# Intel-HLS/GenomicsDB

Hardware: AMD Instinct MI355X
Metric: combined-gVCF positions/sec (higher is better)
Workload: dtype u8/int32

## Files before the change

### __graft_entry__.py

```python
import os
import sys

ROOT = os.path.dirname(os.path.abspath(__file__))
sys.path.insert(0, ROOT)
sys.path.insert(0, os.path.join(ROOT, "tests"))


def build():
    from genomicsdb_amd import build as b
    lib = b.build_native(verbose=True)
    b.build_oracle()
    b.build_hostsim()
    b.build_hostsim_variants()
    b.build_hostsim_import()
    b.build_hostsim_inflate()
    b.build_hostsim_import_bcf()
    b.build_hostsim_import_csv()
    b.build_hostsim_dispatch()
    b.build_hostsim_merge()
    b.build_hostsim_merge_files()
    b.build_hostsim_split()
    b.build_hostsim_histogram()
    b.build_hostsim_index()
    b.build_hostsim_vcfdiff()
    b.build_hostsim_import_stream()
    b.build_hostsim_columns()
    b.build_jni_importer_harness()
    from genomicsdb_amd import synth
    synth.lib()
    import genomicsdb_amd
    from genomicsdb_amd import _lib
    L = _lib.lib()
    for s in _lib.SYMBOLS:
        getattr(L, s)
    print("built", lib)


def smoke():
    import helpers
    from golden_cases import CASES
    import genomicsdb_amd
    case = [c for c in CASES if c[0] == "t6_7_8_vcf_at_0"][0]
    name, callsets, vid, ov, golden, mode = case
    cells = helpers.cells_for(callsets, vid)
    q, pb = helpers.query_json(callsets, vid, ov, mode)
    want, _, _ = helpers.oracle_run(q, cells)
    s = genomicsdb_amd.GenomicsDBQueryStream(query_json=q, cells=cells, buffer_capacity=4096)
    got = s.read()
    s.close()
    assert got == want, "device output differs from the oracle"
    assert got == helpers.golden_text(golden)
    print("smoke ok: %d bytes, bit-exact vs oracle and reference golden" % len(got))


if __name__ == "__main__":
    build()
    if len(sys.argv) > 1 and sys.argv[1] == "smoke":
        smoke()
```

### genomicsdb_amd/build.py

```python
import os
import subprocess
import sys

PKG = os.path.dirname(os.path.abspath(__file__))
ROOT = os.path.dirname(PKG)
CSRC = os.path.join(PKG, "csrc")
OBJ = os.path.join(ROOT, "build", "obj")
LIB = os.path.join(PKG, "libgenomicsdb_amd.so")
TOOL = os.path.join(PKG, "gt_mpi_gather")
TOOLS = {"gt_mpi_gather": TOOL, "vcf2tiledb": os.path.join(PKG, "vcf2tiledb"), "test_genomicsdb_importer": os.path.join(PKG, "test_genomicsdb_importer"),
         "vcf_histogram": os.path.join(PKG, "vcf_histogram"), "vcfdiff": os.path.join(PKG, "vcfdiff")}

SOURCES = [
    "kernels/gdb_pipeline.hip",
    "kernels/gdb_bgzf.hip",
    "kernels/gdb_import.hip",
    "kernels/gdb_import_stream.hip",
    "kernels/gdb_inflate.hip",
    "kernels/gdb_merge.hip",
    "kernels/gdb_split.hip",
    "kernels/gdb_histogram.hip",
    "kernels/gdb_index.hip",
    "kernels/gdb_vcfdiff.hip",
    "kernels/gdb_columns.hip",
# ... 149 lines not shown
    d = os.path.join(ROOT, "tests", "hostsim_index")
    subprocess.check_call(["make", "-s", "-C", d])
    return os.path.join(d, "libhostsim_index.so"), os.path.join(d, "hostsim_index")


def build_hostsim_vcfdiff():
    d = os.path.join(ROOT, "tests", "hostsim_vcfdiff")
    subprocess.check_call(["make", "-s", "-C", d])
    return os.path.join(d, "hostsim_vcfdiff")


def build_hostsim_columns():
    d = os.path.join(ROOT, "tests", "hostsim_columns")
    subprocess.check_call(["make", "-s", "-C", d])
    return os.path.join(d, "libhostsim_columns.so"), os.path.join(d, "hostsim_columns_main")


def build_hostsim_inflate():
    subprocess.check_call(["make", "-s", "-C", os.path.join(ROOT, "tests", "hostsim_inflate")])
    return os.path.join(ROOT, "tests", "hostsim_inflate", "libhostsim_inflate.so")


def build_hostsim_tile_inflate():
    d = os.path.join(ROOT, "tests", "hostsim_tile_inflate")
    subprocess.check_call(["make", "-s", "-C", d])
    return os.path.join(d, "libhostsim_tile_inflate.so"), os.path.join(d, "tile_inflate_fuzz")


def build_hostsim_dispatch():
    subprocess.check_call(["make", "-s", "-C", os.path.join(ROOT, "tests", "hostsim_dispatch")])
    return os.path.join(ROOT, "tests", "hostsim_dispatch", "libhostsim_dispatch.so")


if __name__ == "__main__":
    print(build_native(verbose=True))
    print(build_oracle())
```

### genomicsdb_amd/csrc/core/gdb_stages.hpp

```cpp
#pragma once
#include "gdb_core.hpp"

#if defined(__HIP_DEVICE_COMPILE__)
#define GDB_ATOMIC_ADD_I32(p, v) atomicAdd((int*)(p), (int)(v))
#define GDB_ATOMIC_OR_U32(p, v) atomicOr((unsigned*)(p), (unsigned)(v))
#define GDB_ATOMIC_ADD_U64(p, v) atomicAdd((unsigned long long*)(p), (unsigned long long)(v))
#else
#define GDB_ATOMIC_ADD_I32(p, v) (*(p) += (v))
#define GDB_ATOMIC_OR_U32(p, v) (*(p) |= (v))
#define GDB_ATOMIC_ADD_U64(p, v) (*(p) += (uint64_t)(v))
#endif

#define GDB_EVENT_SENTINEL 0xFFFFFFFFFFFFFFFFull

GDB_HD void stage_eff_end(const FragmentView& fr, const CellMeta& cm, const int64_t* perm, int64_t j, int64_t* rm_begin, int64_t* span, uint32_t* err) {
  const int64_t C = fr.ncells;
  const int64_t c = perm[j];
  int64_t eff = fr.end[c];
  if (j + 1 < C) {
    const int64_t nx = perm[j + 1];
    if (fr.row[nx] == fr.row[c] && fr.begin[nx] <= eff) {
      eff = fr.begin[nx] - 1;
      if (!(cm.cflags[c] & (GDB_CF_DELETION | GDB_CF_REFBLOCK))) *err |= GDB_ERR_OVERLAP_NOT_REFBLOCK_OR_DELETION;
    }
// ... 128 lines not shown
    keys[base + (k - klo)] = (uint64_t)k * (uint64_t)nrows + (uint64_t)fr.row[c];
    vals[base + (k - klo)] = c;
  }
  (void)lut_len;
}
GDB_HD int64_t stage_heavy_base(const uint64_t* sorted_keys, int64_t T, int64_t nrows, int64_t k) {
  const uint64_t want = (uint64_t)k * (uint64_t)nrows;
  int64_t lo = 0, hi = T;
  while (lo < hi) { int64_t mid = (lo + hi) >> 1; if (sorted_keys[mid] < want) lo = mid + 1; else hi = mid; }
  return lo;
}

struct RowIndex {
  const int64_t* row_ptr;
  const int64_t* rm_cell;
  const int64_t* rm_begin;
};
struct RowWalker {
  int64_t j, j_begin, j_end;
  GDB_HD void init(const RowIndex& ri, int32_t row, int64_t s0) {
    j_begin = ri.row_ptr[row]; j_end = ri.row_ptr[row + 1];
    int64_t lo = j_begin, hi = j_end;
    while (lo < hi) { int64_t mid = (lo + hi) >> 1; if (ri.rm_begin[mid] <= s0) lo = mid + 1; else hi = mid; }
    j = lo - 1;
  }
  GDB_HD int64_t live(const RowIndex& ri, const CellMeta& cm, int64_t s) {
    while (j + 1 < j_end && ri.rm_begin[j + 1] <= s) ++j;
    if (j < j_begin) return -1;
    const int64_t c = ri.rm_cell[j];
    return (s <= cm.eff_end[c]) ? c : -1;
  }
};

GDB_HD RecordInfo load_record_info(const SiteOut& so, const HeavyLists& hl, int64_t k) {
  RecordInfo ri;
  ri.num_merged = so.num_alleles[k];
  ri.rflags = so.rflags[k];
  ri.fmt_mask = so.fmt_mask[k];
  ri.hbase = hl.base[k];
  ri.hend = hl.base[k + 1];
  return ri;
}
```

### genomicsdb_amd/csrc/kernels/gdb_assembly_choice.hpp

```cpp
#pragma once
#include <algorithm>
#include <cstdint>
#include <cstdlib>

namespace genomicsdb_amd {

constexpr int kAsmRows = 64;
constexpr int kWaveLds = 8 * 1024;
constexpr int kCooperativeEntry = 512;

enum { kSizeKernelPlain = 0, kSizeKernel3x8 = 1, kSizeKernel3x16 = 2, kSizeKernelPieces = 3, kSizeKernelEvents = 4 };
enum { kPageKernelWrite = 1, kPageKernelWrite2 = 2, kPageKernelWrite3 = 3, kPageKernelEvents = 4, kPageKernelBcf = 5 };
constexpr int page_kernel_code(int size_kernel, int page_kernel, int waves, int coop_u, int lds_bytes) {
  return size_kernel * 100000 + page_kernel * 10000 + waves * 1000 + coop_u * 100 + lds_bytes / 1024;
}

struct AssemblyKnobs {
  int run, run_w, run_w2, run_f;
  uint64_t resolved_budget_bytes;
  bool events; int ev_run;
  int asm_path;
  int size3_rounds;
  bool size3_check;
  bool res_compact;
  bool res_chunk_major;
  int write_waves;
  bool write_image_set; int write_image_kb;
  int order_block_log2;
  bool coop_unroll, xcd_aware;
  int page_priority;

  int image_kb(uint64_t avg_chunk_bytes) const { return write_image_set ? write_image_kb : avg_chunk_bytes && avg_chunk_bytes <= 3400 ? 4 : 8; }
  bool page_priority_on(bool engine_asks) const { return page_priority >= 0 ? page_priority == 1 : engine_asks; }
};

typedef const char* (*KnobLookup)(const char* name);

inline bool res_layout_chunk_major(KnobLookup get) { const char* e = get("GDBAMD_RES_LAYOUT"); return e && *e == '1'; }

inline AssemblyKnobs read_assembly_knobs(KnobLookup get) {
  const auto num = [get](const char* name, int unset, int lo, int hi) { const char* e = get(name); return e && *e ? std::max(lo, std::min(hi, atoi(e))) : unset; };
  const auto on = [get](const char* name) { const char* e = get(name); return e && *e && *e != '0'; };
  const auto not_off = [get](const char* name) { const char* e = get(name); return !(e && *e == '0'); };
  const int any = 0x7fffffff;
  AssemblyKnobs k{};
  const int size3 = num("GDBAMD_SIZE3", 8, -any, any);
  k.size3_rounds = size3 == 0 ? 0 : size3 >= 16 ? 16 : 8;
  k.run = num("GDBAMD_RUN", k.size3_rounds ? 128 : 64, 1, any);
  k.run_w = num("GDBAMD_RUN_W", 32, 1, any);
  k.run_w2 = num("GDBAMD_RUN_W2", 64, 1, any);
  k.run_f = num("GDBAMD_RUN_F", 128, 1, any);
  const char* mb = get("GDBAMD_RESOLVED_MB");
  k.resolved_budget_bytes = mb && *mb ? (uint64_t)atoll(mb) << 20 : (uint64_t)32 << 30;
  k.events = on("GDBAMD_EVENTS");
  k.ev_run = num("GDBAMD_EV_RUN", 32, 1, 64);
  k.asm_path = num("GDBAMD_ASM_PATH", 0, 0, 3);
  k.size3_check = on("GDBAMD_SIZE3_CHECK");
  k.res_compact = !k.size3_check && not_off("GDBAMD_RES_COMPACT");
  k.res_chunk_major = res_layout_chunk_major(get);
  k.write_waves = num("GDBAMD_WRITE_WAVES", 1, -any, any);
  const char* image = get("GDBAMD_WRITE_IMAGE_KB");
  k.write_image_set = image && *image;
  k.write_image_kb = k.write_image_set ? atoi(image) : 0;
  k.order_block_log2 = num("GDBAMD_ORDER_BLOCK_LOG2", 12, 0, 30);
  k.coop_unroll = not_off("GDBAMD_COOP_UNROLL");
  k.xcd_aware = not_off("GDBAMD_XCD_AWARE");
  const char* prio = get("GDBAMD_PAGE_PRIORITY");
  k.page_priority = prio && (*prio == '0' || *prio == '1') ? *prio - '0' : -1;
  return k;
}

inline int size_kernel_for(const AssemblyKnobs& k, int run) {
  return k.size3_rounds == 0 || run > 64 * 1024 ? kSizeKernelPlain : k.size3_rounds >= 16 ? kSizeKernel3x16 : kSizeKernel3x8;
}

struct IntervalFacts { bool bcf_mode; int64_t P; int32_t N; bool untabled_records, any_over255; };

struct AssemblySizing {
  bool bcf_mode;
  int asm_path;
  bool piece_path;
  int size_kernel;
  int run, frun, evrun;
  bool use_events;
  bool resolved_whole;
  bool res_compact;
  bool chunk_major;
  int resolved_entry_bytes;
  int64_t res_rows(int64_t rows) const { return chunk_major ? rows : 0; }
};

inline AssemblySizing choose_sizing(const AssemblyKnobs& k, const IntervalFacts& f) {
  AssemblySizing s{};
  s.bcf_mode = f.bcf_mode;
  const uint64_t nchunks = (uint64_t)((f.N + kAsmRows - 1) / kAsmRows), entry = 8;
  s.asm_path = k.events ? 0 : (f.bcf_mode && (k.asm_path & 1)) ? 2 : k.asm_path;
  if (s.asm_path == 3 && f.untabled_records) s.asm_path = 0;
  s.piece_path = s.asm_path == 1 || s.asm_path == 3;
  s.run = k.run; s.frun = k.run_f; s.evrun = k.ev_run;
  const bool events_fit_blocks = k.events && ((1 << k.order_block_log2) % k.ev_run) == 0;
  s.resolved_whole = !s.piece_path && (f.bcf_mode || ((uint64_t)f.P * nchunks * kAsmRows * entry <= k.resolved_budget_bytes && !events_fit_blocks));
// ... 55 lines not shown
```

### genomicsdb_amd/csrc/kernels/gdb_pipeline.hip

```cpp
#include <hip/hip_runtime.h>

#include <fcntl.h>
#include <sys/stat.h>
#include <unistd.h>
#include <zlib.h>

#include <algorithm>
#include <cstdio>
#include <cstdlib>
#include <chrono>
#include <cstring>
#include <memory>
#include <mutex>
#include <thread>
#include <vector>

#include <rocprim/device/device_radix_sort.hpp>
#include <rocprim/device/device_reduce.hpp>
#include <rocprim/device/device_scan.hpp>
#include <rocprim/iterator/reverse_iterator.hpp>

#include "../core/gdb_stages.hpp"
#include "../core/gdb_bcf.hpp"
#include "../core/gdb_calls.hpp"
// ... 1132 lines not shown
  const bool is_long = l > inline_max;
  if (desc) desc[s] = is_long ? make_uint2(kOverflowBit | ovf16[s], l) : make_uint2((uint32_t)s * (kSlotStride / 16), l);
  if (tag_pool && (is_long || l == 0u)) *reinterpret_cast<uint2*>(tag_pool + (size_t)s * kSlotStride + kSlotTagAt) = make_uint2(is_long ? (kOverflowBit | ovf16[s]) : 0u, l);
}

struct __attribute__((aligned(16))) WalkCell {
  int64_t eff_end;
  uint64_t aux;
  int32_t k_lo, k_hi;
  uint32_t base;
  uint32_t flags;
};
constexpr uint32_t kWalkHeavy = 1u;
constexpr int kWalkChunksShift = 1;
constexpr uint32_t kWalkChunksMask = 7u;
__device__ __forceinline__ uint32_t inline_chunks(uint32_t len) { return len <= (uint32_t)kInlineText ? min((len + 15u) >> 4, kWalkChunksMask) : 0u; }
__global__ void k_walk_static(const int64_t* perm, const int32_t* row, const int64_t* row_ptr, int32_t N, const int64_t* eff_end, const uint32_t* cflags, int64_t C, WalkCell* walk, int64_t* inv) {
  const int64_t j = (int64_t)blockIdx.x * blockDim.x + threadIdx.x;
  WalkCell w;
  w.aux = 0; w.k_lo = -1; w.k_hi = -1; w.base = 0;
  if (j < C) {
    const int64_t c = perm[j];
    const int64_t at = j + row[c];
    w.eff_end = eff_end[c]; w.flags = (cflags[c] & GDB_CF_HEAVY) ? kWalkHeavy : 0u;
    walk[at] = w;
    inv[c] = at;
  } else if (j < C + N) {
    const int64_t r = j - C;
    w.eff_end = INT64_MIN; w.flags = 0;
    walk[row_ptr[r + 1] + r] = w;
  }
}
__global__ void k_walk_window(const int64_t* inv, const uint32_t* cflags, const int64_t* hoff, const int32_t* k_lo, const int32_t* k_hi, const uint32_t* tbase, const uint64_t* tmask,
                              const uint32_t* slot_len, uint32_t light_base, uint32_t heavy_base, int64_t c_base, int64_t n, uint32_t epoch, WalkCell* walk) {
  const int64_t i = (int64_t)blockIdx.x * blockDim.x + threadIdx.x;
  if (i >= n) return;
  const int64_t c = c_base + i;
  WalkCell* w = walk + inv[c];
  const bool heavy = (cflags[c] & GDB_CF_HEAVY) != 0;
  uint32_t chunks = 0;
  if (k_lo[c] >= 0) {
    const uint32_t first = heavy ? heavy_base + (uint32_t)hoff[i] : light_base + tbase[i];
    const uint32_t cnt = heavy ? (uint32_t)(k_hi[c] - k_lo[c] + 1) : (uint32_t)__popcll(tmask[i]);
    for (uint32_t q = 0; q < cnt; ++q) chunks = max(chunks, inline_chunks(slot_len[first + q]));
  }
  const uint4 tail = make_uint4((uint32_t)k_lo[c], (uint32_t)k_hi[c], heavy ? (uint32_t)hoff[i] : tbase[i], (epoch << 8) | (chunks << kWalkChunksShift) | (heavy ? kWalkHeavy : 0u));
  w->aux = heavy ? 0ull : tmask[i];
  *reinterpret_cast<uint4*>(&w->k_lo) = tail;
}

struct AsmCtx {
  const int64_t* row_ptr;
  const int64_t* rm_begin;
  const WalkCell* walk;
  const int64_t* rec_start;
  const uint8_t* rtype;
  const uint32_t* prefix_len;
  const uint2* desc;
  const char* pool;
  const uint32_t* ubase;
  uint32_t light_base, heavy_base, row_base;
  int32_t nrows;
};

struct SlotWalker {
  int64_t j, j_end, next_begin, cur_end;
  uint64_t aux;
  uint32_t base;
  int32_t k_lo, row_;
  bool heavy;
  __device__ __forceinline__ void load(const AsmCtx& a) {
    const WalkCell w = a.walk[j + row_];
    next_begin = (j + 1 < j_end) ? a.rm_begin[j + 1] : INT64_MAX;
    cur_end = w.eff_end; aux = w.aux; base = w.base; k_lo = w.k_lo; heavy = (w.flags & kWalkHeavy) != 0;
  }
  __device__ __forceinline__ void init(const AsmCtx& a, int32_t row, int64_t s0) {
    row_ = row;
    const int64_t j_begin = a.row_ptr[row];
    j_end = a.row_ptr[row + 1];
    int64_t lo = j_begin, hi = j_end;
    while (lo < hi) { const int64_t mid = (lo + hi) >> 1; if (a.rm_begin[mid] <= s0) lo = mid + 1; else hi = mid; }
    j = lo - 1;
    if (j >= j_begin) load(a);
    else { cur_end = INT64_MIN; heavy = false; aux = 0; base = 0; k_lo = 0; next_begin = (j + 1 < j_end) ? a.rm_begin[j + 1] : INT64_MAX; }
  }
  __device__ __forceinline__ void advance(const AsmCtx& a, int64_t s) { while (next_begin <= s) { ++j; load(a); } }
  __device__ __forceinline__ uint32_t slot(const AsmCtx& a, int64_t k, int64_t s, uint32_t t, int32_t row) const {
    const bool dead = s > cur_end;
    if (!dead && heavy) return a.heavy_base + base + (uint32_t)(k - (int64_t)k_lo);
    if (t == kUntabledType) return a.row_base + a.ubase[k] * (uint32_t)a.nrows + (uint32_t)row;
    if (dead) return t;
    return a.light_base + base + (uint32_t)__popcll(aux & ((1ull << t) - 1ull));
  }
};

__device__ __forceinline__ void settle_loads() { __builtin_amdgcn_s_waitcnt(0x0F70); }
struct SlotCopy {
  gdb_lds_char* dst;
  __attribute__((address_space(3))) uint32_t* dw;
  __attribute__((address_space(3))) uint32_t* scrap;
  uint32_t n, h, nw, carry, head_word;
  __device__ __forceinline__ void begin(gdb_lds_char* d, uint32_t len, gdb_lds_char* scrap_word) {
    dst = d; n = len;
    h = (4u - ((uint32_t)(uintptr_t)d & 3u)) & 3u;
    if (h > n) h = n;
    nw = (n - h + 3u) >> 2;
    dw = (__attribute__((address_space(3))) uint32_t*)(d + h);
    scrap = (__attribute__((address_space(3))) uint32_t*)scrap_word;
    carry = 0; head_word = 0;
  }
  __device__ __forceinline__ void put(uint32_t m, uint32_t v) const { *((m < nw) ? dw + m : scrap) = v; }
  __device__ __forceinline__ void chunk(uint32_t q, const uint4& x) {
    if (q == 0) head_word = x.x;
    const uint32_t m1 = q << 2;
    put(m1 - 1u, __builtin_amdgcn_alignbyte(x.x, carry, h));
// ... 37 lines not shown
  __device__ __forceinline__ uint2 load(int64_t at) const {
    if (off) return make_uint2(off[at], (uint32_t)len8[at]);
    return wide[at];
  }
};
__global__ void __launch_bounds__(kAsmRows)
k_assemble_size(AsmCtx a, const int32_t* __restrict__ order, int64_t n, int32_t N, int nchunks, int run, uint64_t* __restrict__ chunk_size,
                ResMatrix resolved, int64_t resolved_base, int64_t res_rows) {
  const int64_t ib = (int64_t)(blockIdx.x / (unsigned)nchunks) * run;
  const int64_t ie = min(n, ib + (int64_t)run);
  const int ch = (int)(blockIdx.x % (unsigned)nchunks);
  const int lane = threadIdx.x;
  const int32_t r = ch * kAsmRows + lane;
  SlotWalker w;
  int64_t prev_k = INT64_MAX;
  uint32_t cur_slot = kNoSlot;
  uint2 cur = make_uint2(0, 0);
  for (int64_t i0 = ib; i0 < ie; i0 += 64) {
    const int cnt = (int)min((int64_t)64, ie - i0);
    int32_t my_k = 0; int64_t my_s = 0; uint32_t my_t = 0; uint64_t my_total = 0;
    if (lane < cnt) {
      my_k = order[i0 + lane];
      my_s = a.rec_start[my_k];
      my_t = a.rtype[my_k];
      if (ch == 0) my_total = a.prefix_len[my_k];
      if (ch == nchunks - 1) my_total += 1;
    }
    for (int jj = 0; jj < cnt; ++jj) {
      const int64_t k = __builtin_amdgcn_readlane(my_k, jj);
      const int64_t s = readlane64(my_s, jj);
      const uint32_t t = (uint32_t)__builtin_amdgcn_readlane((int)my_t, jj);
      uint2 d = make_uint2(0, 0);
      if (r < N) {
        if (k < prev_k) w.init(a, r, s); else w.advance(a, s);
        const uint32_t sl = w.slot(a, k, s, t, r);
        if (sl != cur_slot) { cur_slot = sl; cur = a.desc[sl]; }
        d = cur;
      }
      prev_k = k;
      if (resolved.any()) resolved.store(res_row(k - resolved_base, ch, nchunks, res_rows) * kAsmRows + lane, d);
      const uint32_t total = wave_total(wave_inclusive_scan_dpp(d.y));
      if (lane == jj) my_total += total;
    }
    if (chunk_size && lane < cnt) chunk_size[(int64_t)my_k * nchunks + ch] = my_total;
  }
}

#ifdef GDBAMD_SIZE3_WAVES
#define GDBAMD_SIZE3_ATTR __attribute__((amdgpu_waves_per_eu(GDBAMD_SIZE3_WAVES)))
#else
#define GDBAMD_SIZE3_ATTR
#endif
template <int R> __global__ void __launch_bounds__(kAsmRows) GDBAMD_SIZE3_ATTR
k_assemble_size3(AsmCtx a, const int32_t* __restrict__ order, int64_t n, int32_t N, int nchunks, int run, uint64_t* __restrict__ chunk_size,
                 ResMatrix resolved, int64_t resolved_base, int64_t res_rows) {
  __shared__ int64_t ss[kAsmRows];
  __shared__ int32_t ks[kAsmRows];
  __shared__ uint32_t diff[kAsmRows + 1];
  __shared__ uint2 pl_d[R * kAsmRows];
  __shared__ uint8_t pl_at[R * kAsmRows];
  const int64_t ib = (int64_t)(blockIdx.x / (unsigned)nchunks) * run;
  const int64_t ie = min(n, ib + (int64_t)run);
  const int ch = (int)(blockIdx.x % (unsigned)nchunks);
  const int lane = threadIdx.x;
  const int32_t r = ch * kAsmRows + lane;
  const bool has_row = r < N;
  SlotWalker w;
  int64_t prev_k = INT64_MAX;
  uint32_t cur_slot = kNoSlot;
  uint2 cur = make_uint2(0, 0);
  for (int64_t i0 = ib; i0 < ie; i0 += 64) {
    const int cnt = (int)min((int64_t)64, ie - i0);
    int32_t my_k = 0; int64_t my_s = INT64_MAX; uint32_t my_t = 0; uint64_t my_total = 0;
    if (lane < cnt) {
      my_k = order[i0 + lane];
      my_s = a.rec_start[my_k];
      my_t = a.rtype[my_k];
      if (ch == 0) my_total = a.prefix_len[my_k];
      if (ch == nchunks - 1) my_total += 1;
    }
    ss[lane] = my_s; ks[lane] = my_k; diff[lane] = 0u;
    if (lane == 0) diff[kAsmRows] = 0u;
    const int32_t left_k = __shfl_up(my_k, 1, 64);
    const uint32_t left_t = (uint32_t)__shfl_up((int)my_t, 1, 64);
    const uint64_t heads = __ballot(lane < cnt && (lane == 0 || my_k < left_k || my_t != left_t));
    __builtin_amdgcn_fence(__ATOMIC_SEQ_CST, "wavefront");
    for (int seg_a = 0; seg_a < cnt;) {
      const uint64_t behind = seg_a + 1 < 64 ? heads >> (seg_a + 1) : 0ull;
      const int seg_b = behind ? seg_a + 1 + (int)__builtin_ctzll(behind) : cnt;
      const int64_t k_a = __builtin_amdgcn_readlane(my_k, seg_a);
      const uint32_t t = (uint32_t)__builtin_amdgcn_readlane((int)my_t, seg_a);
      if (k_a < prev_k && has_row) w.init(a, r, readlane64(my_s, seg_a));
      for (int ra = seg_a; ra < seg_b; ra += R) {
        const int rb = min(seg_b, ra + R);
        int pos = ra, np = 0;
        while (__any((int)(pos < rb))) {
          if (pos < rb) {
            uint2 d = make_uint2(0, 0);
            int e = rb;
            if (has_row) {
              const int64_t s = ss[pos];
              const int64_t k = ks[pos];
              w.advance(a, s);
              const uint32_t sl = w.slot(a, k, s, t, r);
              if (sl != cur_slot) { cur_slot = sl; cur = a.desc[sl]; }
              d = cur;
              const bool dead = s > w.cur_end;
              if (t == kUntabledType || (!dead && w.heavy)) e = pos + 1;
              else {
                const int64_t x = dead ? w.next_begin - 1 : min(w.cur_end, w.next_begin - 1);
                int lo = pos + 1, hi = rb;
                while (lo < hi) { const int mid = (lo + hi) >> 1; if (ss[mid] > x) hi = mid; else lo = mid + 1; }
                e = lo;
              }
            }
            pl_d[np * kAsmRows + lane] = d;
            pl_at[np * kAsmRows + lane] = (uint8_t)pos;
            ++np;
            if (chunk_size && d.y) { atomicAdd(&diff[pos], d.y); atomicAdd(&diff[e], 0u - d.y); }
            pos = e;
          }
        }
        __builtin_amdgcn_fence(__ATOMIC_SEQ_CST, "wavefront");
        if (resolved.any()) {
          int q = 0, nxt = ra;
// ... 765 lines not shown
};
constexpr uint32_t kEvLenBits = 20, kEvLenMask = (1u << kEvLenBits) - 1u;

__global__ void __launch_bounds__(kAsmRows)
k_assemble_size_ev(AsmCtx a, const int32_t* __restrict__ order, int64_t n, int32_t N, int nchunks, int run, uint64_t* __restrict__ chunk_size, EventBuf eb, uint32_t* err) {
  const int64_t ib = (int64_t)(blockIdx.x / (unsigned)nchunks) * run;
  const int64_t ie = min(n, ib + (int64_t)run);
  const int ch = (int)(blockIdx.x % (unsigned)nchunks);
  const int lane = threadIdx.x;
  const int32_t r = ch * kAsmRows + lane;
  const int64_t b = blockIdx.x;
  uint2* __restrict__ my_ev = eb.ev + b * (int64_t)run * kAsmRows;
  uint32_t nev = 0;
  SlotWalker w;
  int64_t prev_k = INT64_MAX;
  uint32_t cur_slot = kNoSlot;
  uint2 cur = make_uint2(0, 0);
  const int cnt = (int)(ie - ib);
  int32_t my_k = 0; int64_t my_s = 0; uint32_t my_t = 0; uint64_t my_total = 0;
  if (lane < cnt) {
    my_k = order[ib + lane];
    my_s = a.rec_start[my_k];
    my_t = a.rtype[my_k];
    if (ch == 0) my_total = a.prefix_len[my_k];
    if (ch == nchunks - 1) my_total += 1;
  }
  for (int jj = 0; jj < cnt; ++jj) {
    const int64_t k = __builtin_amdgcn_readlane(my_k, jj);
    const int64_t s = readlane64(my_s, jj);
    const uint32_t t = (uint32_t)__builtin_amdgcn_readlane((int)my_t, jj);
    uint2 d = make_uint2(0, 0);
    bool changed = false;
    if (r < N) {
      if (k < prev_k) w.init(a, r, s); else w.advance(a, s);
      const uint32_t sl = w.slot(a, k, s, t, r);
      if (sl != cur_slot) { cur_slot = sl; const uint2 nd = a.desc[sl]; changed = nd.x != cur.x || nd.y != cur.y; cur = nd; }
      d = cur;
    }
    prev_k = k;
    if (jj == 0) eb.init[b * kAsmRows + lane] = d;
    else {
      const uint64_t m = __ballot(changed);
      if (m) {
        if (changed) {
          const uint32_t rank = (uint32_t)__popcll(m & ((1ull << lane) - 1ull));
          my_ev[nev + rank] = make_uint2(d.x, (d.y & kEvLenMask) | ((uint32_t)lane << kEvLenBits) | ((uint32_t)jj << 26));
          if (d.y > kEvLenMask) atomicOr(err, (uint32_t)GDB_ERR_INTERNAL);
        }
        nev += (uint32_t)__popcll(m);
      }
    }
    const uint32_t total = wave_total(wave_inclusive_scan_dpp(d.y));
    if (lane == jj) my_total += total;
  }
  if (lane < cnt) chunk_size[(int64_t)my_k * nchunks + ch] = my_total;
  if (lane == 0) eb.count[b] = nev;
}

__device__ __forceinline__ u32x4 sload_x4(const void* p) { u32x4 v; asm volatile("s_load_dwordx4 %0, %1, 0x0" : "=s"(v) : "s"(p) : "memory"); return v; }
__device__ __forceinline__ uint64_t sload_x2(const void* p) { uint64_t v; asm volatile("s_load_dwordx2 %0, %1, 0x0" : "=s"(v) : "s"(p) : "memory"); return v; }
__device__ __forceinline__ void swait(uint64_t& a) { asm volatile("s_waitcnt lgkmcnt(0)" : "+s"(a) : : "memory"); }
__device__ __forceinline__ void swait(u32x4& a, u32x4& b, u32x4& c, u32x4& d, u32x4& e) { asm volatile("s_waitcnt lgkmcnt(0)" : "+s"(a), "+s"(b), "+s"(c), "+s"(d), "+s"(e) : : "memory"); }
__device__ __forceinline__ uint32_t wlane(uint32_t sval, uint32_t l, uint32_t old) {
  uint32_t keep;
  asm volatile("s_mov_b32 %1, m0\n\ts_mov_b32 m0, %3\n\tv_writelane_b32 %0, %2, m0\n\ts_mov_b32 m0, %1" : "+v"(old), "=&s"(keep) : "s"(sval), "s"(l));
  return old;
}
// ... 1044 lines not shown
  DevBuf<int32_t> diff, first_record_at; DevBuf<uint64_t> diff_packed; DevBuf<int64_t> heavy_count, hoff;
  DevBuf<uint64_t> inc_keys, inc_keys_sorted; DevBuf<int64_t> inc_vals, inc_vals_sorted, hbase;
  DevBuf<uint32_t> lut_len, i2m_off; DevBuf<int8_t> i2m, gt_override; DevBuf<uint8_t> iflags;
  DevBuf<uint8_t> num_alleles, rflags; DevBuf<uint32_t> fmt_mask, prefix_len; DevBuf<char> site_staging, spill_buf; DevBuf<int32_t> spill_chunk;
  DevBuf<uint64_t> chunk_size, chunk_off, rec_off; DevBuf<unsigned long long> max_record;
  std::unique_ptr<BgzfDeviceCompressor> bgzf;
  void queue_compression(int ai, char* arena, uint64_t page_bytes) {
    if (!hp.bgzf || page_bytes == 0) return;
    if (!bgzf) { bgzf.reset(new BgzfDeviceCompressor); bgzf->set_text(!hp.plan.bcf_mode); bgzf->set_bcf2(hp.plan.bcf_mode != 0); }
    bgzf->enqueue(ai, arena, page_bytes, arena, (void*)stream);
  }
  DevBuf<unsigned int> slot_bump;
  bool long_texts_seen = false;
  uint64_t pool_ovf_need = 0;
  DevBuf<char> arena[2], temp;
  DevBuf<uint32_t> err; DevBuf<int32_t> counters;
  DevBuf<uint32_t> site_key, site_key_sorted; DevBuf<int32_t> site_ord_in, site_ord;
  int ctx_slot = -1;
  DevBuf<char> calls_names, calls_text; DevBuf<int32_t> calls_name_off; DevBuf<uint64_t> calls_len, calls_off; bool calls_names_ready = false; DevBuf<int64_t> calls_array_row; size_t calls_array_row_n = 0;
  DevBuf<int64_t> var_cell, var_end, var_iota, var_sorted, var_run, var_order; DevBuf<uint64_t> var_key, var_key_sorted, var_leader; uint64_t variants_bytes = 0;
  hipEvent_t ev_prep[4] = {nullptr, nullptr, nullptr, nullptr};
  hipEvent_t ev_page[2][4] = {{nullptr, nullptr, nullptr, nullptr}, {nullptr, nullptr, nullptr, nullptr}};
  hipEvent_t arena_release[2] = {nullptr, nullptr};
  struct HostBlock { uint64_t q[80]; uint32_t page_err[2]; } *hb = nullptr;
  DevBuf<SiteCtx> d_sx;
  DevBuf<uint64_t> med_keys, med_keys_sorted; DevBuf<uint32_t> med_idx, med_idx_sorted;
  DevBuf<int32_t> big_index, big_list; DevBuf<uint32_t> big_value; DevBuf<uint8_t> big_ok;
  DevBuf<unsigned long long> remap_total;
  DevBuf<int32_t> huge_index, huge_list; DevBuf<HugeSiteOut> huge_out; DevBuf<SiteCtx> d_sx0;
  DevBuf<uint32_t> slot_cell; DevBuf<float> tie_buf; DevBuf<unsigned long long> tie_used; DevBuf<uint32_t> scalar_pre;
  DevBuf<unsigned long long> type_hkeys; DevBuf<int32_t> type_hrep, type_rep; DevBuf<uint8_t> type_hid, rtype;
  DevBuf<WalkCell> walk; DevBuf<int64_t> walk_inv;
  DevBuf<int32_t> jhint;
  DevBuf<unsigned long long> dbg_counters;
  DevBuf<uint32_t> pl_cnt, pl_ofs; DevBuf<PieceEntry> plist;
  uint32_t walk_epoch = 0;
  DevBuf<uint8_t> raw_cells; DevBuf<uint64_t> raw_off; DevBuf<int32_t> raw_row_map, raw_qrow; DevBuf<uint32_t> raw_keep, raw_dest, raw_len, raw_voff, raw_mark, raw_mdest;
  DevBuf<int64_t> raw_begin, raw_end;
  DevBuf<uint64_t> walk_bitmap, walk_pos, walk_out; DevBuf<uint32_t> walk_wcount, walk_wrank, walk_succ, walk_jump_a, walk_jump_b, walk_flag, walk_dest; DevBuf<uint8_t> walk_reach;
  DevBuf<int64_t> walk_cut; DevBuf<unsigned long long> walk_kept_bytes;
  DevBuf<uint8_t> inflate_in, inflate_out, inflate_scratch, inflate_status; DevBuf<uint64_t> inflate_off; DevBuf<uint32_t> inflate_want;
  DevBuf<long long> carry_last; DevBuf<uint64_t> carry_keys, carry_sorted; int64_t carried_cells = 0;
  DevBuf<uint2> chk_resolved; DevBuf<uint64_t> chk_sizes; DevBuf<unsigned long long> chk_count;
  DevBuf<uint2> resolved;
  DevBuf<uint32_t> res_off; DevBuf<uint8_t> res_len8;
  DevBuf<unsigned int> slot_over;
  DevBuf<uint32_t> type_occ;
  DevBuf<uint32_t> untabled, ubase; DevBuf<int32_t> urec, iota, order; DevBuf<uint32_t> order_keys, order_keys_sorted;
  DevBuf<uint64_t> tmask; DevBuf<uint32_t> nslots, tbase, slot_len, slot_units, slot_off; DevBuf<uint2> slot_desc; DevBuf<char> pool, pool_ovf;
  bool classified = false;
  uint64_t fragment_generation = 0;
  struct Part { FragmentView v; std::vector<size_t> data_bytes; std::vector<void*> bufs; };
  std::vector<Part> parts;
  std::vector<int> col_elem_size; std::vector<bool> col_var; std::vector<int> col_fixed_num;
  std::unique_ptr<DevicePipeline::FragmentFile> ff;
  struct IntervalState {
    bool active = false;
    int64_t P = 0, kp = 0;
    int nchunks = 0;
    uint64_t max_record_bytes = 0, total_bytes = 0;
    float write_kernel_ms = 0;
    std::vector<uint64_t> rec_off;
    IntervalStats stats;
    SiteCtx sx; EntryCtx ex; RowIndex ri; SiteOut so; RecordTable rec; AsmCtx ac; PieceCtx pc2;
    AssemblyKnobs knobs{};
    AssemblySizing sz{};
// ... 1724 lines not shown
      S.pool_ovf.p = np; S.pool_ovf.cap = ncap;
    }
    stt.pool_ovf = S.pool_ovf.p;
    stt.bump_cap = shard_units_of(S.pool_ovf.cap);
    STAGE("k_slots<1>");
    GDB_SLOT_KERNELS(1, kStripWords);
  } else if (left_texts > 0) {
    hipLaunchKernelGGL(k_slot_units, dim3(blocks_for((int64_t)NS)), dim3(kBlock), 0, st, S.slot_len.p, (int64_t)NS, S.slot_units.p, stt.inline_max);
    S.excl_scan(S.slot_units.p, S.slot_off.p, (size_t)NS);
    pool_units = (uint64_t)S.read_back_sum(S.slot_off.p + (NS - 1), S.slot_units.p + (NS - 1));
    if (pool_units >= (uint64_t)kOverflowBit) throw GenomicsDBDeviceException("entry text overflow pool exceeds 32 GiB: split the query interval");
    S.pool_ovf.ensure((size_t)pool_units * 16 + 64);
    stt.pool_ovf = S.pool_ovf.p;
    stt.bump_cap = 0;
    STAGE("k_slots<1>");
    GDB_SLOT_KERNELS(1, kStripWords);
  }
#undef GDB_SLOT_KERNELS
  S.long_texts_seen = long_texts * 16 > NS;
  S.pool_ovf_need = std::max<uint64_t>(S.pool_ovf_need, shard_need);
  const AssemblySizing sz = S.iv.sz = choose_sizing(S.iv.knobs, IntervalFacts{pl.bcf_mode != 0, P, N, UR > 0, any_over255});
  const int asm_path = sz.asm_path;
  hipLaunchKernelGGL(k_slot_desc, dim3(blocks_for((int64_t)NS)), dim3(kBlock), 0, st, S.slot_len.p, S.slot_off.p, (int64_t)NS, asm_path == 1 ? (uint2*)nullptr : S.slot_desc.p,
                     pl.bcf_mode ? (char*)nullptr : S.pool.p, stt.inline_max);
  stats.num_record_types = ntypes;
  stats.resolved_entry_bytes = sz.resolved_entry_bytes;
  stats.num_text_slots = (int64_t)NS;
  stats.text_pool_bytes = (int64_t)(NS * kSlotStride + pool_units * 16);
  STAGE("k_walk_window");
  if (++S.walk_epoch >= (1u << 24)) {
    hipLaunchKernelGGL(k_walk_static, dim3(blocks_for(C + N)), dim3(kBlock), 0, st, S.perm.p, fr.row, S.row_ptr.p, N, S.eff_end.p, S.cflags.p, C, S.walk.p, S.walk_inv.p);
    S.walk_epoch = 1;
  }
  hipLaunchKernelGGL(k_walk_window, dim3(blocks_for(CW)), dim3(kBlock), 0, st, S.walk_inv.p, S.cflags.p, S.hoff.p, S.k_lo.p, S.k_hi.p, S.tbase.p, S.tmask.p,
                     (const uint32_t*)S.slot_len.p, (uint32_t)kMaxTypes, (uint32_t)(kMaxTypes + SL), c_base, CW, S.walk_epoch, S.walk.p);
  AsmCtx ac{S.row_ptr.p, S.rm_begin.p, S.walk.p, S.rstart.p, S.rtype.p, S.prefix_len.p, S.slot_desc.p, S.pool.p, S.ubase.p,
            (uint32_t)kMaxTypes, (uint32_t)(kMaxTypes + SL), (uint32_t)(kMaxTypes + SL + (uint64_t)T), N};
  S.jhint.ensure((size_t)((P + kHintStep - 1) / kHintStep) * (size_t)N + 1);
  PieceCtx pc2{S.row_ptr.p, S.rm_begin.p, S.walk.p, S.rstart.p, S.rtype.p, S.ubase.p, S.type_occ.p, S.slot_len.p, S.prefix_len.p, S.jhint.p,
               (uint32_t)kMaxTypes, (uint32_t)(kMaxTypes + SL), (uint32_t)(kMaxTypes + SL + (uint64_t)T), S.walk_epoch, N, P};
  const int run = sz.run, frun = sz.frun, evrun = sz.evrun;
  const dim3 size_grid((unsigned)((P + run - 1) / run) * (unsigned)nchunks);
  STAGE("k_assemble_size");
  if (!sz.piece_path) S.order_by_type(0, P, S.iv.knobs.order_block_log2);
  if (sz.resolved_whole) {
    if (sz.res_compact) { S.res_off.ensure((size_t)P * nchunks * kAsmRows); S.res_len8.ensure((size_t)P * nchunks * kAsmRows); }
    else S.resolved.ensure((size_t)P * nchunks * kAsmRows);
  }
  S.max_record.ensure(1);
  HIP_CHECK(hipMemsetAsync(S.max_record.p, 0, sizeof(unsigned long long), st));
  BcfLayout lay{nullptr, nullptr, nullptr, nullptr};
  const int bcf_F = std::max(1, pl.n_format);
  const uint64_t size2_units = (uint64_t)((P + kSizeBlock - 1) / kSizeBlock) * (uint64_t)nchunks;
  if (asm_path != 0 && size2_units >= (1ull << 31)) throw GenomicsDBDeviceException("more than 2^31 (record block, sample chunk) units in one interval: split the query interval");
  const unsigned fill_units = (unsigned)(((P + frun - 1) / frun) * nchunks);
  if (pl.bcf_mode) {
    if (asm_path == 2) {
      hipLaunchKernelGGL(k_size2, dim3((unsigned)size2_units), dim3(kAsmRows), 0, st, pc2, nchunks, S.chunk_size.p);
      hipLaunchKernelGGL(k_fill2, dim3(fill_units), dim3(kAsmRows), 0, st, pc2, (const uint2*)S.slot_desc.p, (const int32_t*)S.order.p, P, nchunks, frun, S.resolved.p, (int64_t)0);
    } else
    launch_assemble_size(S, st, sz.size_kernel, size_grid, ac, S.order.p, P, N, nchunks, run, (uint64_t*)nullptr, 0, S.res_view(), (int64_t)0, (int64_t)0);
    S.bcf_part.ensure(nchunk_total * (size_t)bcf_F + 1); S.bcf_fmeta.ensure((size_t)P * bcf_F + 1); S.bcf_foff.ensure((size_t)P * bcf_F + 1); S.bcf_lindiv.ensure((size_t)P + 1);
    S.bcf_rec_size.ensure((size_t)P + 2);
    lay = BcfLayout{S.bcf_fmeta.p, S.bcf_foff.p, S.bcf_lindiv.p, S.bcf_rec_size.p};
    STAGE("k_bcf_field_meta");
    hipLaunchKernelGGL(k_bcf_field_meta, dim3((unsigned)(((P + kBcfRun - 1) / kBcfRun) * nchunks)), dim3(kAsmRows), 0, st, S.res_view(), (const char*)S.pool.p,
                       (const char*)S.pool_ovf.p, (const uint32_t*)S.fmt_mask.p, (const int32_t*)S.order.p, P, nchunks, bcf_F, S.bcf_part.p);
    hipLaunchKernelGGL(k_bcf_layout, dim3(blocks_for(P)), dim3(kBlock), 0, st, pl, (const uint32_t*)S.bcf_part.p, (const uint32_t*)S.fmt_mask.p, (const uint32_t*)S.prefix_len.p, P,
                       nchunks, bcf_F, lay);
    HIP_CHECK(hipMemsetAsync(S.bcf_rec_size.p + P, 0, sizeof(uint64_t), st));
// ... 239 lines not shown
```

Measured before the change: 40.34 million.

## Seed slot walker with per-row walk hints instead of binary search

The walk-window kernel now records, for every 128-record block and row, the smallest row-relative cell index overlapping that block, using atomicMin into a hint table reset to a sentinel each interval. SlotWalker::init reads this hint and steps forward linearly from it rather than binary-searching rm_begin over the row's cells. This is meant to cut the cost of re-seeding the walker in the assembly kernels. In exchange it adds a memset, atomics per cell across the blocks it spans, and a linear scan that can get long when many cells fall between hint points.

```diff
diff --git a/__graft_entry__.py b/__graft_entry__.py
--- a/__graft_entry__.py
+++ b/__graft_entry__.py
@@ -25,6 +25,7 @@
     b.build_hostsim_vcfdiff()
     b.build_hostsim_import_stream()
     b.build_hostsim_columns()
+    b.build_hostsim_walk_hint()
     b.build_jni_importer_harness()
     from genomicsdb_amd import synth
     synth.lib()
diff --git a/genomicsdb_amd/build.py b/genomicsdb_amd/build.py
--- a/genomicsdb_amd/build.py
+++ b/genomicsdb_amd/build.py
@@ -205,6 +205,12 @@
     return os.path.join(ROOT, "tests", "hostsim_dispatch", "libhostsim_dispatch.so")
 
 
+def build_hostsim_walk_hint():
+    d = os.path.join(ROOT, "tests", "hostsim_walk_hint")
+    subprocess.check_call(["make", "-s", "-C", d])
+    return os.path.join(d, "walk_hint_main"), os.path.join(d, "walk_hint_main_san")
+
+
 if __name__ == "__main__":
     print(build_native(verbose=True))
     print(build_oracle())
diff --git a/genomicsdb_amd/csrc/core/gdb_stages.hpp b/genomicsdb_amd/csrc/core/gdb_stages.hpp
--- a/genomicsdb_amd/csrc/core/gdb_stages.hpp
+++ b/genomicsdb_amd/csrc/core/gdb_stages.hpp
@@ -184,6 +184,25 @@
   }
 };
 
+constexpr int kWalkHintStep = 128;
+constexpr int32_t kWalkHintNone = 0x7FFFFFFF;
+GDB_HD bool walk_hint_rows(int32_t k_lo, int32_t k_hi, int64_t& h0, int64_t& h1) {
+  if (k_lo < 0 || k_hi < k_lo) return false;
+  h0 = ((int64_t)k_lo + kWalkHintStep - 1) / kWalkHintStep;
+  h1 = (int64_t)k_hi / kWalkHintStep;
+  return h0 <= h1;
+}
+GDB_HD int64_t walk_start(const int64_t* rm_begin, int64_t j_begin, int64_t j_end, int32_t hint, int64_t s) {
+  if (hint == kWalkHintNone) {
+    int64_t lo = j_begin, hi = j_end;
+    while (lo < hi) { const int64_t mid = (lo + hi) >> 1; if (rm_begin[mid] <= s) lo = mid + 1; else hi = mid; }
+    return lo - 1;
+  }
+  int64_t j = j_begin + hint;
+  while (j + 1 < j_end && rm_begin[j + 1] <= s) ++j;
+  return j;
+}
+
 GDB_HD RecordInfo load_record_info(const SiteOut& so, const HeavyLists& hl, int64_t k) {
   RecordInfo ri;
   ri.num_merged = so.num_alleles[k];
diff --git a/genomicsdb_amd/csrc/kernels/gdb_assembly_choice.hpp b/genomicsdb_amd/csrc/kernels/gdb_assembly_choice.hpp
--- a/genomicsdb_amd/csrc/kernels/gdb_assembly_choice.hpp
+++ b/genomicsdb_amd/csrc/kernels/gdb_assembly_choice.hpp
@@ -29,6 +29,7 @@
   int order_block_log2;
   bool coop_unroll, xcd_aware;
   int page_priority;
+  bool walk_hint;
 
   int image_kb(uint64_t avg_chunk_bytes) const { return write_image_set ? write_image_kb : avg_chunk_bytes && avg_chunk_bytes <= 3400 ? 4 : 8; }
   bool page_priority_on(bool engine_asks) const { return page_priority >= 0 ? page_priority == 1 : engine_asks; }
@@ -67,6 +68,7 @@
   k.xcd_aware = not_off("GDBAMD_XCD_AWARE");
   const char* prio = get("GDBAMD_PAGE_PRIORITY");
   k.page_priority = prio && (*prio == '0' || *prio == '1') ? *prio - '0' : -1;
+  k.walk_hint = not_off("GDBAMD_WALK_HINT");
   return k;
 }
 
diff --git a/genomicsdb_amd/csrc/kernels/gdb_pipeline.hip b/genomicsdb_amd/csrc/kernels/gdb_pipeline.hip
--- a/genomicsdb_amd/csrc/kernels/gdb_pipeline.hip
+++ b/genomicsdb_amd/csrc/kernels/gdb_pipeline.hip
@@ -1188,11 +1188,19 @@
   }
 }
 __global__ void k_walk_window(const int64_t* inv, const uint32_t* cflags, const int64_t* hoff, const int32_t* k_lo, const int32_t* k_hi, const uint32_t* tbase, const uint64_t* tmask,
-                              const uint32_t* slot_len, uint32_t light_base, uint32_t heavy_base, int64_t c_base, int64_t n, uint32_t epoch, WalkCell* walk) {
+                              const uint32_t* slot_len, uint32_t light_base, uint32_t heavy_base, int64_t c_base, int64_t n, uint32_t epoch, WalkCell* walk,
+                              const int32_t* row, const int64_t* row_ptr, int32_t nrows, int32_t* hint) {
   const int64_t i = (int64_t)blockIdx.x * blockDim.x + threadIdx.x;
   if (i >= n) return;
   const int64_t c = c_base + i;
   WalkCell* w = walk + inv[c];
+  int64_t h0, h1;
+  if (hint && walk_hint_rows(k_lo[c], k_hi[c], h0, h1)) {
+    const int32_t r = row[c];
+    const int64_t rel = inv[c] - r - row_ptr[r];
+    if (r >= 0 && r < nrows && rel >= 0 && rel < (int64_t)kWalkHintNone)
+      for (int64_t h = h0; h <= h1; ++h) atomicMin(&hint[h * nrows + r], (int32_t)rel);
+  }
   const bool heavy = (cflags[c] & GDB_CF_HEAVY) != 0;
   uint32_t chunks = 0;
   if (k_lo[c] >= 0) {
@@ -1217,6 +1225,7 @@
   const uint32_t* ubase;
   uint32_t light_base, heavy_base, row_base;
   int32_t nrows;
+  const int32_t* hint;
 };
 
 struct SlotWalker {
@@ -1230,13 +1239,12 @@
     next_begin = (j + 1 < j_end) ? a.rm_begin[j + 1] : INT64_MAX;
     cur_end = w.eff_end; aux = w.aux; base = w.base; k_lo = w.k_lo; heavy = (w.flags & kWalkHeavy) != 0;
   }
-  __device__ __forceinline__ void init(const AsmCtx& a, int32_t row, int64_t s0) {
+  __device__ __forceinline__ void init(const AsmCtx& a, int32_t row, int64_t k, int64_t s0) {
     row_ = row;
     const int64_t j_begin = a.row_ptr[row];
     j_end = a.row_ptr[row + 1];
-    int64_t lo = j_begin, hi = j_end;
-    while (lo < hi) { const int64_t mid = (lo + hi) >> 1; if (a.rm_begin[mid] <= s0) lo = mid + 1; else hi = mid; }
-    j = lo - 1;
+    const int32_t hint = a.hint ? a.hint[(k / kWalkHintStep) * a.nrows + row] : kWalkHintNone;
+    j = walk_start(a.rm_begin, j_begin, j_end, hint, s0);
     if (j >= j_begin) load(a);
     else { cur_end = INT64_MIN; heavy = false; aux = 0; base = 0; k_lo = 0; next_begin = (j + 1 < j_end) ? a.rm_begin[j + 1] : INT64_MAX; }
   }
@@ -1340,7 +1348,7 @@
       const uint32_t t = (uint32_t)__builtin_amdgcn_readlane((int)my_t, jj);
       uint2 d = make_uint2(0, 0);
       if (r < N) {
-        if (k < prev_k) w.init(a, r, s); else w.advance(a, s);
+        if (k < prev_k) w.init(a, r, k, s); else w.advance(a, s);
         const uint32_t sl = w.slot(a, k, s, t, r);
         if (sl != cur_slot) { cur_slot = sl; cur = a.desc[sl]; }
         d = cur;
@@ -1398,7 +1406,7 @@
       const int seg_b = behind ? seg_a + 1 + (int)__builtin_ctzll(behind) : cnt;
       const int64_t k_a = __builtin_amdgcn_readlane(my_k, seg_a);
       const uint32_t t = (uint32_t)__builtin_amdgcn_readlane((int)my_t, seg_a);
-      if (k_a < prev_k && has_row) w.init(a, r, readlane64(my_s, seg_a));
+      if (k_a < prev_k && has_row) w.init(a, r, k_a, readlane64(my_s, seg_a));
       for (int ra = seg_a; ra < seg_b; ra += R) {
         const int rb = min(seg_b, ra + R);
         int pos = ra, np = 0;
@@ -2230,7 +2238,7 @@
     uint2 d = make_uint2(0, 0);
     bool changed = false;
     if (r < N) {
-      if (k < prev_k) w.init(a, r, s); else w.advance(a, s);
+      if (k < prev_k) w.init(a, r, k, s); else w.advance(a, s);
       const uint32_t sl = w.slot(a, k, s, t, r);
       if (sl != cur_slot) { cur_slot = sl; const uint2 nd = a.desc[sl]; changed = nd.x != cur.x || nd.y != cur.y; cur = nd; }
       d = cur;
@@ -3341,6 +3349,7 @@
   DevBuf<unsigned long long> type_hkeys; DevBuf<int32_t> type_hrep, type_rep; DevBuf<uint8_t> type_hid, rtype;
   DevBuf<WalkCell> walk; DevBuf<int64_t> walk_inv;
   DevBuf<int32_t> jhint;
+  DevBuf<int32_t> walk_hint;
   DevBuf<unsigned long long> dbg_counters;
   DevBuf<uint32_t> pl_cnt, pl_ofs; DevBuf<PieceEntry> plist;
   uint32_t walk_epoch = 0;
@@ -5131,10 +5140,18 @@
     hipLaunchKernelGGL(k_walk_static, dim3(blocks_for(C + N)), dim3(kBlock), 0, st, S.perm.p, fr.row, S.row_ptr.p, N, S.eff_end.p, S.cflags.p, C, S.walk.p, S.walk_inv.p);
     S.walk_epoch = 1;
   }
+  int32_t* walk_hint = nullptr;
+  if (S.iv.knobs.walk_hint) {
+    const size_t nhint = (size_t)((P + kWalkHintStep - 1) / kWalkHintStep) * (size_t)N;
+    S.walk_hint.ensure(nhint + 1);
+    HIP_CHECK(hipMemsetD32Async((hipDeviceptr_t)S.walk_hint.p, kWalkHintNone, nhint, st));
+    walk_hint = S.walk_hint.p;
+  }
   hipLaunchKernelGGL(k_walk_window, dim3(blocks_for(CW)), dim3(kBlock), 0, st, S.walk_inv.p, S.cflags.p, S.hoff.p, S.k_lo.p, S.k_hi.p, S.tbase.p, S.tmask.p,
-                     (const uint32_t*)S.slot_len.p, (uint32_t)kMaxTypes, (uint32_t)(kMaxTypes + SL), c_base, CW, S.walk_epoch, S.walk.p);
+                     (const uint32_t*)S.slot_len.p, (uint32_t)kMaxTypes, (uint32_t)(kMaxTypes + SL), c_base, CW, S.walk_epoch, S.walk.p,
+                     fr.row, (const int64_t*)S.row_ptr.p, N, walk_hint);
   AsmCtx ac{S.row_ptr.p, S.rm_begin.p, S.walk.p, S.rstart.p, S.rtype.p, S.prefix_len.p, S.slot_desc.p, S.pool.p, S.ubase.p,
-            (uint32_t)kMaxTypes, (uint32_t)(kMaxTypes + SL), (uint32_t)(kMaxTypes + SL + (uint64_t)T), N};
+            (uint32_t)kMaxTypes, (uint32_t)(kMaxTypes + SL), (uint32_t)(kMaxTypes + SL + (uint64_t)T), N, walk_hint};
   S.jhint.ensure((size_t)((P + kHintStep - 1) / kHintStep) * (size_t)N + 1);
   PieceCtx pc2{S.row_ptr.p, S.rm_begin.p, S.walk.p, S.rstart.p, S.rtype.p, S.ubase.p, S.type_occ.p, S.slot_len.p, S.prefix_len.p, S.jhint.p,
                (uint32_t)kMaxTypes, (uint32_t)(kMaxTypes + SL), (uint32_t)(kMaxTypes + SL + (uint64_t)T), S.walk_epoch, N, P};
```

Result: no change. 40.67 million, median of 6 (+0.8%).
